# double125/MADTP

Hardware: AMD Instinct MI355X
Metric: images/sec forward, BLIP-base NLVR2 p=0.5 b64; pruned-token index match (higher is better)
Workload: dtype bf16

## Files before the change

madtp_amd/csrc/attention.hip:

```cpp
#include "common.h"
#include "internal.h"
#include <map>
#include <mutex>
#include <stdlib.h>

namespace {

struct AttnArgs {
    const char* q; const char* k; const char* v; char* out; const float* mask;
    float* colsum; float* p0; float* onorm;
    int B, H, Nq, Nk, ldq, ldk, ldv, ldo, nrt;
    float scale;
    const int* kvidx;
    const char* q2; const char* k2; const char* v2; char* out2; const float* mask2; int pair;
    const float* mask_qk; int ld_mqk;
    unsigned* hm_ws; int* hm_tick;
    int kvb;
    float* o_part;
    const int32_t* n_dev;
    int dev_q_only;
    int split_dim; int* range_flag;
};
#define ATTN_DEV_DIMS(a)                                   \
    if ((a).n_dev) {                                       \
// ... 225 lines not shown
    if constexpr (SCORES) {
        if (gridDim.z == 2) {
            const size_t slot = ((size_t)b * gridDim.x + blockIdx.x) * 4 + wave;
            unsigned* mine = a.hm_ws + ((slot * 2 + blockIdx.z) * (2 * HM_MAX_NT)) * 64 + lane;
#pragma unroll
            for (int t = 0; t < NT; ++t)
#pragma unroll
                for (int r = 0; r < 4; ++r)
                    __hip_atomic_store(mine + (4 * t + r) * 64, __float_as_uint(pmax[t][r]), __ATOMIC_RELAXED, __HIP_MEMORY_SCOPE_AGENT);
            asm volatile("s_waitcnt vmcnt(0)" ::: "memory");
            int old = 0;
            if (lane == 0) old = __hip_atomic_fetch_add(a.hm_tick + slot, 1, __ATOMIC_RELAXED, __HIP_MEMORY_SCOPE_AGENT);
            old = __builtin_amdgcn_readfirstlane(old);
            if (old == 0) return;
            if (lane == 0) __hip_atomic_store(a.hm_tick + slot, 0, __ATOMIC_RELAXED, __HIP_MEMORY_SCOPE_AGENT);
            const unsigned* theirs = a.hm_ws + ((slot * 2 + (1 - blockIdx.z)) * (2 * HM_MAX_NT)) * 64 + lane;
#pragma unroll
            for (int t = 0; t < NT; ++t)
#pragma unroll
                for (int r = 0; r < 4; ++r)
                    pmax[t][r] = fmaxf(pmax[t][r], __uint_as_float(__hip_atomic_load(theirs + (4 * t + r) * 64, __ATOMIC_RELAXED,
                                                                                      __HIP_MEMORY_SCOPE_AGENT)));
        }
        if (active) {
            const int i = i0 + l16;
            const bool valid = i >= 1 && i < a.Nq;
            float* dst = a.colsum + ((size_t)b * a.nrt + rt) * a.Nk;
#pragma unroll
            for (int t = 0; t < NT; ++t)
#pragma unroll
                for (int r = 0; r < 4; ++r) {
                    const float v = row16_sum(valid ? pmax[t][r] : 0.f);
                    const int j = 16 * t + 4 * g + r;
                    if (l16 == 0 && j < a.Nk) dst[j] = v;
                }
        }
    }
}

template <int NT, bool SCORES>
__global__ __launch_bounds__(256) void attn_f16s_kernel(AttnArgs a) {
    ATTN_DEV_DIMS(a)
    constexpr int PITCH = NT <= 15 ? 160 : 144;
    constexpr int NKP = NT * 16;
    constexpr int NC = (NT + 1) / 2;
    constexpr int VR = NC * 32;
    extern __shared__ __attribute__((aligned(16))) char smem[];
    char* K0 = smem;
    char* K1 = K0 + NKP * PITCH;
    char* V0 = K1 + NKP * PITCH;
    char* V1 = V0 + VR * PITCH;

    const int tid = threadIdx.x, lane = tid & 63, wave = tid >> 6;
    const int l16 = lane & 15, g = lane >> 4;
    const int b = blockIdx.y;
    const int bkv = a.kvidx ? a.kvidx[b] : b;
    const int rt = blockIdx.x * 4 + wave;
    const int i0 = rt * 16;
    const bool active = i0 < a.Nq;
    const int irow = min(i0 + l16, a.Nq - 1);

    f32x4 pmax[NT];
    if constexpr (SCORES) {
#pragma unroll
        for (int t = 0; t < NT; ++t) pmax[t] = (f32x4){0.f, 0.f, 0.f, 0.f};
    }
    f32x4 mk[NT];
#pragma unroll
    for (int t = 0; t < NT; ++t)
#pragma unroll
        for (int r = 0; r < 4; ++r) {
            const int j = 16 * t + 4 * g + r;
            mk[t][r] = j < a.Nk ? (a.mask ? a.mask[(size_t)b * a.Nk + j] : 0.f) : -INFINITY;
            if (a.mask_qk && j < a.Nk) mk[t][r] += a.mask_qk[(size_t)irow * a.ld_mqk + j];
        }
    if constexpr (VR > NKP) {
        for (int idx = tid; idx < (VR - NKP) * (PITCH / 16); idx += 256) {
            *(uint4*)(V0 + NKP * PITCH + idx * 16) = make_uint4(0, 0, 0, 0);
            *(uint4*)(V1 + NKP * PITCH + idx * 16) = make_uint4(0, 0, 0, 0);
        }
    }

    constexpr int NLD = NT;
    constexpr bool PREFETCH = NLD <= 8;
    uint4 kreg[PREFETCH ? NLD : 1], vreg[PREFETCH ? NLD : 1];
    auto fetch = [&](int h) {
#pragma unroll
        for (int i = 0; i < NLD; ++i) {
            const int idx = tid + 256 * i;
            const int row = idx >> 4, c = idx & 15;
            kreg[i] = make_uint4(0, 0, 0, 0);
            vreg[i] = make_uint4(0, 0, 0, 0);
            if (row < a.Nk) {
                const size_t grow = (size_t)bkv * a.kvb + row;
                kreg[i] = *(const uint4*)(a.k + (grow * a.ldk + h * 64) * 4 + c * 16);
                vreg[i] = *(const uint4*)(a.v + (grow * a.ldv + h * 64) * 4 + c * 16);
            }
        }
    };
    auto put = [&](int idx, uint4 kv, uint4 vv) {
        const int row = idx >> 4, c = idx & 15;
        f16x4 h4, l4;
        split_f16x4(__builtin_bit_cast(f32x4, kv), h4, l4);
        *(f16x4*)(K0 + row * PITCH + c * 8) = h4;
        *(f16x4*)(K1 + row * PITCH + c * 8) = l4;
        split_f16x4(__builtin_bit_cast(f32x4, vv), h4, l4);
        *(f16x4*)(V0 + row * PITCH + c * 8) = h4;
        *(f16x4*)(V1 + row * PITCH + c * 8) = l4;
    };
    if constexpr (PREFETCH) {
        if ((int)blockIdx.z < a.H) fetch(blockIdx.z);
    }
    constexpr float LO = 1.0f / F16S_LO_SCALE;
    for (int h = blockIdx.z; h < a.H; h += gridDim.z) {
        __syncthreads();
        if constexpr (PREFETCH) {
#pragma unroll
            for (int i = 0; i < NLD; ++i) put(tid + 256 * i, kreg[i], vreg[i]);
        } else {
            for (int idx = tid; idx < NKP * 16; idx += 256) {
                const int row = idx >> 4, c = idx & 15;
                uint4 kv = make_uint4(0, 0, 0, 0), vv = make_uint4(0, 0, 0, 0);
                if (row < a.Nk) {
                    const size_t grow = (size_t)bkv * a.kvb + row;
                    kv = *(const uint4*)(a.k + (grow * a.ldk + h * 64) * 4 + c * 16);
                    vv = *(const uint4*)(a.v + (grow * a.ldv + h * 64) * 4 + c * 16);
                }
                put(idx, kv, vv);
            }
        }
        __syncthreads();
        if constexpr (PREFETCH) {
            if (h + (int)gridDim.z < a.H) fetch(h + gridDim.z);
        }
        if (!active) continue;

        f16x8 qh[2], ql[2];
        {
            const char* qp = a.q + (((size_t)b * a.Nq + irow) * a.ldq + h * 64) * 4 + g * 32;
#pragma unroll
            for (int kk = 0; kk < 2; ++kk) {
                u32x4 p0, p1;
                split_f16x8(*(const f32x4*)(qp + kk * 128), *(const f32x4*)(qp + kk * 128 + 16), p0, p1);
                qh[kk] = __builtin_bit_cast(f16x8, p0);
                ql[kk] = __builtin_bit_cast(f16x8, p1);
            }
        }

        f32x4 sc[NT];
#pragma unroll
        for (int t = 0; t < NT; ++t) {
            const int off = (16 * t + l16) * PITCH + g * 16;
            const f16x8 kh0 = *(const f16x8*)(K0 + off), kh1 = *(const f16x8*)(K0 + off + 64);
            const f16x8 kl0 = *(const f16x8*)(K1 + off), kl1 = *(const f16x8*)(K1 + off + 64);
            const f32x4 z = (f32x4){0.f, 0.f, 0.f, 0.f};
            f32x4 hi = __builtin_amdgcn_mfma_f32_16x16x32_f16(kh0, qh[0], z, 0, 0, 0);
            hi = __builtin_amdgcn_mfma_f32_16x16x32_f16(kh1, qh[1], hi, 0, 0, 0);
            f32x4 lo = __builtin_amdgcn_mfma_f32_16x16x32_f16(kh0, ql[0], z, 0, 0, 0);
            lo = __builtin_amdgcn_mfma_f32_16x16x32_f16(kh1, ql[1], lo, 0, 0, 0);
            lo = __builtin_amdgcn_mfma_f32_16x16x32_f16(kl0, qh[0], lo, 0, 0, 0);
            lo = __builtin_amdgcn_mfma_f32_16x16x32_f16(kl1, qh[1], lo, 0, 0, 0);
#pragma unroll
            for (int r = 0; r < 4; ++r) sc[t][r] = fmaf(lo[r], LO, hi[r]);
        }

        float m = -INFINITY;
#pragma unroll
        for (int t = 0; t < NT; ++t)
#pragma unroll
            for (int r = 0; r < 4; ++r) {
                const float v = __fadd_rn(__fmul_rn(sc[t][r], a.scale), mk[t][r]);
                sc[t][r] = v;
                m = fmaxf(m, v);
            }
        m = rows4_max(m);
        float sum = 0.f;
#pragma unroll
        for (int t = 0; t < NT; ++t)
#pragma unroll
            for (int r = 0; r < 4; ++r) {
                const float p = expf(sc[t][r] - m);
                sc[t][r] = p;
                sum += p;
            }
        sum = rows4_sum(sum);
#pragma unroll
        for (int t = 0; t < NT; ++t)
#pragma unroll
            for (int r = 0; r < 4; ++r) {
                const float p = sc[t][r] / sum;
                sc[t][r] = p;
                if constexpr (SCORES) pmax[t][r] = fmaxf(pmax[t][r], p);
            }
        if constexpr (SCORES) {
            if (i0 == 0 && l16 == 0) {
                float* dst = a.p0 + ((size_t)b * a.H + h) * a.Nk;
#pragma unroll
                for (int t = 0; t < NT; ++t)
#pragma unroll
                    for (int r = 0; r < 4; ++r) {
                        const int j = 16 * t + 4 * g + r;
                        if (j < a.Nk) dst[j] = sc[t][r];
                    }
            }
        }

        f32x4 oh[4], ol[4];
#pragma unroll
        for (int dt = 0; dt < 4; ++dt) { oh[dt] = (f32x4){0.f, 0.f, 0.f, 0.f}; ol[dt] = (f32x4){0.f, 0.f, 0.f, 0.f}; }
#pragma unroll
        for (int c = 0; c < NC; ++c) {
            const f32x4 t1 = (2 * c + 1 < NT) ? sc[2 * c + 1 < NT ? 2 * c + 1 : 0] : (f32x4){0.f, 0.f, 0.f, 0.f};
            u32x4 pp0, pp1;
            split_f16x8(sc[2 * c], t1, pp0, pp1);
            const f16x8 ph = __builtin_bit_cast(f16x8, pp0), pl = __builtin_bit_cast(f16x8, pp1);
            const int voff = (32 * c + 4 * g + (l16 >> 2)) * PITCH + 8 * (l16 & 3);
#pragma unroll
            for (int dt = 0; dt < 4; ++dt) {
                const bf16x8 vh = cat_bf16x4(lds_read_tr16(V0 + voff + dt * 32), lds_read_tr16(V0 + voff + 16 * PITCH + dt * 32));
                const bf16x8 vl = cat_bf16x4(lds_read_tr16(V1 + voff + dt * 32), lds_read_tr16(V1 + voff + 16 * PITCH + dt * 32));
                oh[dt] = __builtin_amdgcn_mfma_f32_16x16x32_f16(__builtin_bit_cast(f16x8, vh), ph, oh[dt], 0, 0, 0);
                ol[dt] = __builtin_amdgcn_mfma_f32_16x16x32_f16(__builtin_bit_cast(f16x8, vh), pl, ol[dt], 0, 0, 0);
                ol[dt] = __builtin_amdgcn_mfma_f32_16x16x32_f16(__builtin_bit_cast(f16x8, vl), ph, ol[dt], 0, 0, 0);
            }
        }

        {
            const int i = i0 + l16;
            f32x4 o[4];
            float n2 = 0.f;
#pragma unroll
            for (int dt = 0; dt < 4; ++dt)
#pragma unroll
                for (int r = 0; r < 4; ++r) {
                    o[dt][r] = fmaf(ol[dt][r], LO, oh[dt][r]);
                    n2 += o[dt][r] * o[dt][r];
                }
            if constexpr (SCORES) n2 = rows4_sum(n2);
            if (i < a.Nq) {
                if (a.split_dim) {
                    _Float16* prow = (_Float16*)a.out + ((size_t)b * a.Nq + i) * a.ldo + h * 64 + 4 * g;
                    bool bad = false;
#pragma unroll
                    for (int dt = 0; dt < 4; ++dt) {
                        f16x4 ph_, pl_;
                        split_f16x4(o[dt], ph_, pl_);
                        *(f16x4*)(prow + dt * 16) = ph_;
                        *(f16x4*)(prow + a.split_dim + dt * 16) = pl_;
                        bad |= f16_range_bad(o[dt]);
                    }
                    f16_range_raise(a.range_flag, bad);
                } else {
                    float* orow = (float*)(a.out + (((size_t)b * a.Nq + i) * a.ldo + h * 64) * 4) + 4 * g;
#pragma unroll
                    for (int dt = 0; dt < 4; ++dt) *(f32x4*)(orow + dt * 16) = o[dt];
                }
                if constexpr (SCORES)
                    if (g == 0) a.onorm[((size_t)b * a.H + h) * a.Nq + i] = sqrtf(n2);
            }
        }
    }

    if constexpr (SCORES) {
        if (gridDim.z == 2) {
            const size_t slot = ((size_t)b * gridDim.x + blockIdx.x) * 4 + wave;
            unsigned* mine = a.hm_ws + ((slot * 2 + blockIdx.z) * (2 * HM_MAX_NT)) * 64 + lane;
#pragma unroll
            for (int t = 0; t < NT; ++t)
#pragma unroll
                for (int r = 0; r < 4; ++r)
                    __hip_atomic_store(mine + (4 * t + r) * 64, __float_as_uint(pmax[t][r]), __ATOMIC_RELAXED, __HIP_MEMORY_SCOPE_AGENT);
            asm volatile("s_waitcnt vmcnt(0)" ::: "memory");
            int old = 0;
            if (lane == 0) old = __hip_atomic_fetch_add(a.hm_tick + slot, 1, __ATOMIC_RELAXED, __HIP_MEMORY_SCOPE_AGENT);
            old = __builtin_amdgcn_readfirstlane(old);
            if (old == 0) return;
            if (lane == 0) __hip_atomic_store(a.hm_tick + slot, 0, __ATOMIC_RELAXED, __HIP_MEMORY_SCOPE_AGENT);
            const unsigned* theirs = a.hm_ws + ((slot * 2 + (1 - blockIdx.z)) * (2 * HM_MAX_NT)) * 64 + lane;
#pragma unroll
            for (int t = 0; t < NT; ++t)
#pragma unroll
                for (int r = 0; r < 4; ++r)
                    pmax[t][r] = fmaxf(pmax[t][r], __uint_as_float(__hip_atomic_load(theirs + (4 * t + r) * 64, __ATOMIC_RELAXED,
                                                                                      __HIP_MEMORY_SCOPE_AGENT)));
        }
        if (active) {
            const int i = i0 + l16;
            const bool valid = i >= 1 && i < a.Nq;
            float* dst = a.colsum + ((size_t)b * a.nrt + rt) * a.Nk;
#pragma unroll
            for (int t = 0; t < NT; ++t)
#pragma unroll
                for (int r = 0; r < 4; ++r) {
                    const float v = row16_sum(valid ? pmax[t][r] : 0.f);
                    const int j = 16 * t + 4 * g + r;
                    if (l16 == 0 && j < a.Nk) dst[j] = v;
                }
        }
    }
}

#ifdef MADTP_TS_TIMING
__device__ long long g_attn_dbg[8];
#define AT_MARK(i) do { if (threadIdx.x == 0 && blockIdx.x == 0 && blockIdx.y == 0 && it == 2) { __builtin_amdgcn_s_waitcnt(0); g_attn_dbg[i] = wall_clock64(); } } while (0)
#else
#define AT_MARK(i)
#endif
template <int NT, bool SCORES, int HS, int RB = 1, bool F16 = false>
__global__ __launch_bounds__(256 * HS * RB, (HS == 1 && RB == 1) ? 2 : 1) void attn_bf16_kernel(AttnArgs a) {
    ATTN_DEV_DIMS(a)
    static_assert(HS == 1 || RB == 1, "head-parity split and two row blocks are alternatives");
    constexpr int NKP = NT * 16;
    constexpr int NC = (NT + 1) / 2;
    constexpr int VR = NC * 32;
    constexpr int STAGE = (NKP + VR) * 128;
    extern __shared__ __attribute__((aligned(16))) char smem[];

    const int tid = threadIdx.x, lane = tid & 63;
    const int wave8 = __builtin_amdgcn_readfirstlane(tid >> 6);
    const int wave = wave8 & 3;
    const int hp = HS == 2 ? wave8 >> 2 : 0;
    const int rb = RB == 2 ? wave8 >> 2 : 0;
    constexpr int NSW = 4 * RB;
    const int swave = RB == 2 ? wave8 : wave;
    char* const ring = smem + hp * 2 * STAGE;
    const int l16 = lane & 15, g = lane >> 4;
    int b = blockIdx.y;
    if (a.pair && b >= a.B) {
        b -= a.B;
        a.q = a.q2; a.k = a.k2; a.v = a.v2; a.out = a.out2; a.mask = a.mask2;
    }
    const int bkv = a.kvidx ? a.kvidx[b] : b;
    const int rt = (blockIdx.x * RB + rb) * 4 + wave;
    const int i0 = rt * 16;
    const bool active = i0 < a.Nq;
    const int irow = min(i0 + l16, a.Nq - 1);

    f32x4 pmax[NT];
    if constexpr (SCORES) {
#pragma unroll
        for (int t = 0; t < NT; ++t) pmax[t] = (f32x4){0.f, 0.f, 0.f, 0.f};
    }
    f32x4 mk[NT];
#pragma unroll
    for (int t = 0; t < NT; ++t)
#pragma unroll
        for (int r = 0; r < 4; ++r) {
            const int j = 16 * t + 4 * g + r;
            mk[t][r] = j < a.Nk ? (a.mask ? a.mask[(size_t)b * a.Nk + j] : 0.f) : -INFINITY;
            if (a.mask_qk && j < a.Nk) mk[t][r] += a.mask_qk[(size_t)irow * a.ld_mqk + j];
            mk[t][r] *= 1.44269504088896341f;
        }
    const float c2 = a.scale * 1.44269504088896341f;

    const int sub = lane >> 3, pos = lane & 7;
    constexpr int NDMA = ((NKP + VR) / 8 + NSW - 1) / NSW;
    const char* srcb[NDMA];
#pragma unroll
    for (int i = 0; i < NDMA; ++i) {
        const int grp = swave + NSW * i;
        const bool is_v = grp >= NKP / 8;
        int row = (is_v ? grp - NKP / 8 : grp) * 8 + sub;
        const int chunk = is_v ? (pos ^ (((row >> 1) & 3) << 1)) : (pos ^ (row & 7));
        row = row < a.Nk ? row : a.Nk - 1;
        srcb[i] = (is_v ? a.v + ((size_t)bkv * a.kvb + row) * a.ldv * 2 : a.k + ((size_t)bkv * a.kvb + row) * a.ldk * 2) + chunk * 16;
    }
    auto stage_head = [&](int h, int st) {
        char* base = ring + st * STAGE;
#pragma unroll
        for (int i = 0; i < NDMA; ++i) {
            const int grp = swave + NSW * i;
            if (grp < (NKP + VR) / 8)
                __builtin_amdgcn_global_load_lds(GLOBAL_PTR(srcb[i] + h * 128), LDS_PTR(base + grp * 1024), 16, 0, 0);
        }
    };
    const char* qbase = a.q + ((size_t)b * a.Nq + irow) * a.ldq * 2 + g * 16;
    auto load_q = [&](int h, bf16x8 (&qq)[2]) {
        const char* qp = qbase + h * 128;
        qq[0] = *(const bf16x8*)qp;
        qq[1] = *(const bf16x8*)(qp + 64);
    };
    int st = 0;
    const int hstep = gridDim.z * HS;
    const int hfirst = blockIdx.z * HS + hp;
    const int niter = (a.H - (int)blockIdx.z * HS + hstep - 1) / hstep;
    bf16x8 qn[2];
    if (hfirst < a.H) {
        stage_head(hfirst, 0);
        load_q(hfirst, qn);
    }
    for (int it = 0; it < niter; ++it, st ^= 1) {
        const int h = hfirst + it * hstep;
        bf16x8 q[2] = {qn[0], qn[1]};
        AT_MARK(0);
        __syncthreads();
        AT_MARK(1);
        if (h + hstep < a.H) {
            stage_head(h + hstep, st ^ 1);
            load_q(h + hstep, qn);
        }
        if (!active || h >= a.H) continue;
        AT_MARK(2);
        const char* Ks = ring + st * STAGE;
        const char* Vs = Ks + NKP * 128;

        f32x4 sc[NT];
#pragma unroll
        for (int t = 0; t < NT; ++t) {
            const int row = 16 * t + l16;
            const bf16x8 k0 = *(const bf16x8*)(Ks + row * 128 + (((0 + g) ^ (row & 7)) << 4));
            const bf16x8 k1 = *(const bf16x8*)(Ks + row * 128 + (((4 + g) ^ (row & 7)) << 4));
            f32x4 acc = (f32x4){0.f, 0.f, 0.f, 0.f};
            acc = mfma_lp<F16>(k0, q[0], acc, 0, 0, 0);
            sc[t] = mfma_lp<F16>(k1, q[1], acc, 0, 0, 0);
        }
        AT_MARK(3);
        float m = -INFINITY;
#pragma unroll
        for (int t = 0; t < NT; ++t)
#pragma unroll
            for (int r = 0; r < 4; ++r) {
                const float v = fmaf(sc[t][r], c2, mk[t][r]);
                sc[t][r] = v;
                m = fmaxf(m, v);
            }
        m = rows4_max(m);
        float sum = 0.f;
#pragma unroll
        for (int t = 0; t < NT; ++t)
#pragma unroll
            for (int r = 0; r < 4; ++r) {
                const float p = __builtin_amdgcn_exp2f(sc[t][r] - m);
                sc[t][r] = p;
                sum += p;
            }
        sum = rows4_sum(sum);
        const float inv = __builtin_amdgcn_rcpf(sum);
#pragma unroll
        for (int t = 0; t < NT; ++t) {
            sc[t] *= inv;
            if constexpr (SCORES) {
#pragma unroll
                for (int r = 0; r < 4; ++r) pmax[t][r] = fmaxf(pmax[t][r], sc[t][r]);
            }
        }
        if constexpr (SCORES) {
            if (i0 == 0) {
                if (l16 == 0) {
                    float* dst = a.p0 + ((size_t)b * a.H + h) * a.Nk;
#pragma unroll
                    for (int t = 0; t < NT; ++t)
#pragma unroll
                        for (int r = 0; r < 4; ++r) {
                            const int j = 16 * t + 4 * g + r;
                            if (j < a.Nk) dst[j] = sc[t][r];
                        }
                }
            }
        }
        AT_MARK(4);
        f32x4 o[4];
#pragma unroll
        for (int dt = 0; dt < 4; ++dt) o[dt] = (f32x4){0.f, 0.f, 0.f, 0.f};
#pragma unroll
        for (int c = 0; c < NC; ++c) {
            const f32x4 hi = (2 * c + 1 < NT) ? sc[2 * c + 1 < NT ? 2 * c + 1 : 0] : (f32x4){0.f, 0.f, 0.f, 0.f};
            const bf16x8 pa = pack_lp8<F16>(sc[2 * c], hi);
            const int vrow = 32 * c + 4 * g + (l16 >> 2);
            const int vkey = ((vrow >> 1) & 3) << 1;
            const char* vr = Vs + vrow * 128 + 8 * (l16 & 1);
#pragma unroll
            for (int dt = 0; dt < 4; ++dt) {
                const int p = ((2 * dt + ((l16 & 3) >> 1)) ^ vkey) << 4;
                const bf16x8 vb = cat_bf16x4(lds_read_tr16(vr + p), lds_read_tr16(vr + 16 * 128 + p));
                o[dt] = mfma_lp<F16>(vb, pa, o[dt], 0, 0, 0);
            }
        }
        AT_MARK(5);
        {
            const int i = i0 + l16;
            float n2 = 0.f;
#pragma unroll
            for (int dt = 0; dt < 4; ++dt)
#pragma unroll
                for (int r = 0; r < 4; ++r) n2 += o[dt][r] * o[dt][r];
            if constexpr (SCORES) {
                n2 = rows4_sum(n2);
            }
            if (i < a.Nq) {
                bf16_t* orow = (bf16_t*)(a.out + (((size_t)b * a.Nq + i) * a.ldo + h * 64) * 2) + 4 * g;
#pragma unroll
                for (int dt = 0; dt < 4; ++dt) *(bf16x4*)(orow + dt * 16) = pack_lp4<F16>(o[dt]);
                if constexpr (SCORES)
                    if (g == 0) a.onorm[((size_t)b * a.H + h) * a.Nq + i] = sqrtf(n2);
            }
        }
        AT_MARK(6);
    }

    if constexpr (SCORES && HS == 2) {
        f32x4* xch = (f32x4*)smem;
        __syncthreads();
        if (hp == 1)
#pragma unroll
            for (int t = 0; t < NT; ++t) xch[(wave * NT + t) * 64 + lane] = pmax[t];
        __syncthreads();
        if (hp == 1) return;
#pragma unroll
        for (int t = 0; t < NT; ++t) {
            const f32x4 o = xch[(wave * NT + t) * 64 + lane];
#pragma unroll
            for (int r = 0; r < 4; ++r) pmax[t][r] = fmaxf(pmax[t][r], o[r]);
        }
    }
    if constexpr (SCORES) {
        if (active) {
            const int i = i0 + l16;
            const bool valid = i >= 1 && i < a.Nq;
            float* dst = a.colsum + ((size_t)b * a.nrt + rt) * a.Nk;
#pragma unroll
            for (int t = 0; t < NT; ++t)
#pragma unroll
                for (int r = 0; r < 4; ++r) {
                    const float v = row16_sum(valid ? pmax[t][r] : 0.f);
                    const int j = 16 * t + 4 * g + r;
                    if (l16 == 0 && j < a.Nk) dst[j] = v;
                }
        }
    }
}

constexpr int SMALL_NW = 12;
template <bool F16>
__global__ __launch_bounds__(64 * SMALL_NW, 1) void attn_bf16_small_kernel(AttnArgs a) {
    __shared__ __attribute__((aligned(16))) char vbuf[SMALL_NW][32 * 128];
    __shared__ float pm[SMALL_NW][2][2][64][4];
    const int tid = threadIdx.x, lane = tid & 63;
    const int wave = __builtin_amdgcn_readfirstlane(tid >> 6);
    const int l16 = lane & 15, g = lane >> 4;
    const int b = blockIdx.x;
    const int N = a.Nk;
    char* Vs = vbuf[wave];
    f32x4 pmax[2][2];
#pragma unroll
    for (int rt = 0; rt < 2; ++rt)
#pragma unroll
        for (int t = 0; t < 2; ++t) pmax[rt][t] = (f32x4){0.f, 0.f, 0.f, 0.f};
    const int nrt = (N + 15) / 16;
    f32x4 mk[2];
#pragma unroll
    for (int t = 0; t < 2; ++t)
#pragma unroll
        for (int r = 0; r < 4; ++r) {
            const int j = 16 * t + 4 * g + r;
            mk[t][r] = (j < N ? (a.mask ? a.mask[(size_t)b * N + j] : 0.f) : -INFINITY) * 1.44269504088896341f;
        }
    const float c2 = a.scale * 1.44269504088896341f;

    for (int h = wave; h < a.H; h += SMALL_NW) {
        {
            const int sub = lane >> 3, pos = lane & 7;
#pragma unroll
            for (int grp = 0; grp < 4; ++grp) {
                int row = grp * 8 + sub;
                const int chunk = pos ^ (((row >> 1) & 3) << 1);
                row = row < N ? row : N - 1;
                *(bf16x8*)(Vs + grp * 1024 + lane * 16) =
                    *(const bf16x8*)(a.v + (((size_t)b * N + row) * a.ldv + h * 64) * 2 + chunk * 16);
            }
        }
        bf16x8 kf[2][2];
#pragma unroll
        for (int t = 0; t < 2; ++t) {
            const int j = min(16 * t + l16, N - 1);
            const char* kp = a.k + (((size_t)b * N + j) * a.ldk + h * 64) * 2 + g * 16;
            kf[t][0] = *(const bf16x8*)kp;
            kf[t][1] = *(const bf16x8*)(kp + 64);
        }
#pragma unroll
        for (int rt = 0; rt < 2; ++rt) {
            if (rt >= nrt) break;
            const int i0 = rt * 16;
            const int irow = min(i0 + l16, N - 1);
            const char* qp = a.q + (((size_t)b * N + irow) * a.ldq + h * 64) * 2 + g * 16;
            const bf16x8 q0 = *(const bf16x8*)qp, q1 = *(const bf16x8*)(qp + 64);
            f32x4 sc[2];
            float m = -INFINITY;
#pragma unroll
            for (int t = 0; t < 2; ++t) {
                f32x4 acc = (f32x4){0.f, 0.f, 0.f, 0.f};
                acc = mfma_lp<F16>(kf[t][0], q0, acc, 0, 0, 0);
                acc = mfma_lp<F16>(kf[t][1], q1, acc, 0, 0, 0);
#pragma unroll
                for (int r = 0; r < 4; ++r) {
                    const float v = fmaf(acc[r], c2, mk[t][r]);
                    acc[r] = v;
                    m = fmaxf(m, v);
                }
                sc[t] = acc;
            }
            m = rows4_max(m);
            float sum = 0.f;
#pragma unroll
            for (int t = 0; t < 2; ++t)
#pragma unroll
                for (int r = 0; r < 4; ++r) { sc[t][r] = __builtin_amdgcn_exp2f(sc[t][r] - m); sum += sc[t][r]; }
            sum = rows4_sum(sum);
            const float inv = __builtin_amdgcn_rcpf(sum);
#pragma unroll
            for (int t = 0; t < 2; ++t) {
                sc[t] *= inv;
#pragma unroll
                for (int r = 0; r < 4; ++r) pmax[rt][t][r] = fmaxf(pmax[rt][t][r], sc[t][r]);
            }
            if (i0 == 0) if (l16 == 0) {
                float* dst = a.p0 + ((size_t)b * a.H + h) * N;
#pragma unroll
                for (int t = 0; t < 2; ++t)
#pragma unroll
                    for (int r = 0; r < 4; ++r) {
                        const int j = 16 * t + 4 * g + r;
                        if (j < N) dst[j] = sc[t][r];
                    }
            }
            const bf16x8 pa = pack_lp8<F16>(sc[0], sc[1]);
            const int vrow = 4 * g + (l16 >> 2);
            const int vkey = ((vrow >> 1) & 3) << 1;
            const char* vr = Vs + vrow * 128 + 8 * (l16 & 1);
            f32x4 o[4];
            float n2 = 0.f;
#pragma unroll
            for (int dt = 0; dt < 4; ++dt) {
                const int p = ((2 * dt + ((l16 & 3) >> 1)) ^ vkey) << 4;
                const bf16x8 vb = cat_bf16x4(lds_read_tr16(vr + p), lds_read_tr16(vr + 16 * 128 + p));
                o[dt] = mfma_lp<F16>(vb, pa, (f32x4){0.f, 0.f, 0.f, 0.f}, 0, 0, 0);
#pragma unroll
                for (int r = 0; r < 4; ++r) n2 += o[dt][r] * o[dt][r];
            }
            n2 = rows4_sum(n2);
            const int i = i0 + l16;
            if (i < N) {
                bf16_t* orow = (bf16_t*)(a.out + (((size_t)b * N + i) * a.ldo + h * 64) * 2) + 4 * g;
#pragma unroll
                for (int dt = 0; dt < 4; ++dt) *(bf16x4*)(orow + dt * 16) = pack_lp4<F16>(o[dt]);
                if (g == 0) a.onorm[((size_t)b * a.H + h) * N + i] = sqrtf(n2);
            }
        }
    }
#pragma unroll
    for (int rt = 0; rt < 2; ++rt)
#pragma unroll
        for (int t = 0; t < 2; ++t)
#pragma unroll
            for (int r = 0; r < 4; ++r) pm[wave][rt][t][lane][r] = pmax[rt][t][r];
    __syncthreads();
    if (wave < nrt) {
        const int rt = wave, i = rt * 16 + l16;
        const bool valid = i >= 1 && i < N;
        float* dst = a.colsum + ((size_t)b * a.nrt + rt) * N;
#pragma unroll
        for (int t = 0; t < 2; ++t)
#pragma unroll
            for (int r = 0; r < 4; ++r) {
                float v = pm[0][rt][t][lane][r];
#pragma unroll
                for (int w = 1; w < SMALL_NW; ++w) v = fmaxf(v, pm[w][rt][t][lane][r]);
                v = row16_sum(valid ? v : 0.f);
                const int j = 16 * t + 4 * g + r;
                if (l16 == 0 && j < N) dst[j] = v;
            }
    }
}

template <int NT, bool SCORES, bool F16>
int launch_attn_bf16(const AttnArgs& a, hipStream_t s) {
    constexpr int NC = (NT + 1) / 2;
    constexpr int HS = (SCORES && NT <= 8) ? 2 : 1;
    constexpr int RB = (SCORES && NT > 8) ? 2 : 1;
    const size_t lds = (size_t)2 * HS * (NT * 16 + NC * 32) * 128;
    MADTP_ENSURE_MAX_LDS((attn_bf16_kernel<NT, SCORES, HS, RB, F16>), lds);
    int gz = 1;
    size_t lds_used = lds;
    if (!SCORES) {
        const int wgs = ((a.Nq + 63) / 64) * a.B;
        gz = wgs >= 512 ? 1 : a.H;
        if (gz == a.H) lds_used = lds / 2;
    }
    hipLaunchKernelGGL((attn_bf16_kernel<NT, SCORES, HS, RB, F16>), dim3((a.Nq + 64 * RB - 1) / (64 * RB), (!SCORES && a.pair) ? 2 * a.B : a.B, gz),
                       dim3(256 * HS * RB), lds_used, s, a);
    MADTP_LAUNCH_CHECK();
    return 0;
}

template <bool SCORES, bool F16 = false>
int dispatch_nt_bf16(const AttnArgs& a, hipStream_t s) {
    const int nt = (a.Nk + 15) / 16;
    if (nt <= 4) return launch_attn_bf16<4, SCORES, F16>(a, s);
    if (nt <= 6) return launch_attn_bf16<6, SCORES, F16>(a, s);
    if (nt <= 8) return launch_attn_bf16<8, SCORES, F16>(a, s);
    if (nt <= 10) return launch_attn_bf16<10, SCORES, F16>(a, s);
    if (nt <= 12) return launch_attn_bf16<12, SCORES, F16>(a, s);
    if (nt <= 13) return launch_attn_bf16<13, SCORES, F16>(a, s);
    if (nt <= 16) return launch_attn_bf16<16, SCORES, F16>(a, s);
    return MADTP_E_SHAPE;
}

template <typename T, int NCH, bool SCORES>
__global__ __launch_bounds__(256, 1) void attn_large_kernel(AttnArgs a) {
    constexpr int ESZ = sizeof(T);
    constexpr int RB = 64 * ESZ + 16;
    constexpr int CPR = 64 * ESZ / 16;
    constexpr int CK = 128;
    constexpr int NT = NCH * 8;
    extern __shared__ __attribute__((aligned(16))) char smem[];
    char* Ks = smem;
    char* Vs = smem + CK * RB;

    const int tid = threadIdx.x, lane = tid & 63, wave = tid >> 6;
    const int l16 = lane & 15, g = lane >> 4;
    const int b = blockIdx.y;
    const int bkv = a.kvidx ? a.kvidx[b] : b;
    const int rt = blockIdx.x * 4 + wave;
    const int i0 = rt * 16;
    const bool active = i0 < a.Nq;
    const int irow = min(i0 + l16, a.Nq - 1);

    f32x4 pmax[SCORES ? NT : 1];
    if constexpr (SCORES) {
#pragma unroll
        for (int t = 0; t < NT; ++t) pmax[t] = (f32x4){0.f, 0.f, 0.f, 0.f};
    }

    auto stage = [&](int h, int c, bool with_v) {
        for (int idx = tid; idx < CK * CPR; idx += 256) {
            const int row = idx / CPR, ch = idx % CPR, j = c * CK + row;
            uint4 kv = make_uint4(0, 0, 0, 0), vv = make_uint4(0, 0, 0, 0);
            if (j < a.Nk) {
                const size_t grow = (size_t)bkv * a.kvb + j;
                kv = *(const uint4*)(a.k + (grow * a.ldk + h * 64) * ESZ + ch * 16);
                if (with_v) vv = *(const uint4*)(a.v + (grow * a.ldv + h * 64) * ESZ + ch * 16);
            }
            *(uint4*)(Ks + row * RB + ch * 16) = kv;
            if (with_v) *(uint4*)(Vs + row * RB + ch * 16) = vv;
        }
    };
    auto scores = [&](int c, const f32x4 (&q)[4], f32x4 (&sc)[8]) {
#pragma unroll
        for (int t = 0; t < 8; ++t) sc[t] = (f32x4){0.f, 0.f, 0.f, 0.f};
#pragma unroll
        for (int s = 0; s < 4; ++s) {
            f32x4 kf[8];
#pragma unroll
            for (int t = 0; t < 8; ++t) kf[t] = load4<T>(Ks + (16 * t + l16) * RB + (4 * s + g) * 4 * ESZ);
#pragma unroll
            for (int e = 0; e < 4; ++e)
#pragma unroll
                for (int t = 0; t < 8; ++t) sc[t] = __builtin_amdgcn_mfma_f32_16x16x4f32(kf[t][e], q[s][e], sc[t], 0, 0, 0);
        }
#pragma unroll
        for (int t = 0; t < 8; ++t)
#pragma unroll
            for (int r = 0; r < 4; ++r) {
                const int j = c * CK + 16 * t + 4 * g + r;
                float v = sc[t][r] * a.scale;
                if (a.mask && j < a.Nk) v += a.mask[(size_t)b * a.Nk + j];
                sc[t][r] = j < a.Nk ? v : -INFINITY;
            }
    };

    for (int h = blockIdx.z; h < a.H; h += gridDim.z) {
        f32x4 q[4];
        {
            const char* qp = a.q + (((size_t)b * a.Nq + irow) * a.ldq + h * 64) * ESZ;
#pragma unroll
            for (int s = 0; s < 4; ++s) q[s] = load4<T>(qp + (4 * s + g) * 4 * ESZ);
        }
        float m = -INFINITY, l = 0.f;
        for (int c = 0; c < NCH; ++c) {
            if (c * CK >= a.Nk) break;
            __syncthreads();
            stage(h, c, false);
            __syncthreads();
            if (!active) continue;
            f32x4 sc[8];
            scores(c, q, sc);
            float cm = -INFINITY;
#pragma unroll
            for (int t = 0; t < 8; ++t)
#pragma unroll
                for (int r = 0; r < 4; ++r) cm = fmaxf(cm, sc[t][r]);
            cm = rows4_max(cm);
            const float mn = fmaxf(m, cm);
            float cs = 0.f;
#pragma unroll
            for (int t = 0; t < 8; ++t)
#pragma unroll
                for (int r = 0; r < 4; ++r) cs += expf(sc[t][r] - mn);
            cs = rows4_sum(cs);
            l = l * expf(m - mn) + cs;
            m = mn;
        }
        f32x4 o[4];
#pragma unroll
        for (int dt = 0; dt < 4; ++dt) o[dt] = (f32x4){0.f, 0.f, 0.f, 0.f};
#pragma unroll
        for (int c = 0; c < NCH; ++c) {
            if (c * CK < a.Nk) {
                __syncthreads();
                stage(h, c, true);
                __syncthreads();
                if (active) {
                    f32x4 sc[8];
                    scores(c, q, sc);
#pragma unroll
                    for (int t = 0; t < 8; ++t) {
#pragma unroll
                        for (int r = 0; r < 4; ++r) {
                            const float p = expf(sc[t][r] - m) / l;
                            sc[t][r] = p;
                            if constexpr (SCORES) pmax[c * 8 + t][r] = fmaxf(pmax[c * 8 + t][r], p);
                        }
                    }
                    if constexpr (SCORES) {
                        if (i0 + l16 == 0) {
                            float* dst = a.p0 + ((size_t)b * a.H + h) * a.Nk;
#pragma unroll
                            for (int t = 0; t < 8; ++t)
#pragma unroll
                                for (int r = 0; r < 4; ++r) {
                                    const int j = c * CK + 16 * t + 4 * g + r;
                                    if (j < a.Nk) dst[j] = sc[t][r];
                                }
                        }
                    }
#pragma unroll
                    for (int t = 0; t < 8; ++t)
#pragma unroll
                        for (int r = 0; r < 4; ++r) {
                            const char* vrow = Vs + (16 * t + 4 * g + r) * RB + l16 * ESZ;
#pragma unroll
                            for (int dt = 0; dt < 4; ++dt)
                                o[dt] = __builtin_amdgcn_mfma_f32_16x16x4f32(sc[t][r], load1<T>(vrow + dt * 16 * ESZ), o[dt], 0, 0, 0);
                        }
                }
            }
        }
        if (active) {
#pragma unroll
            for (int r = 0; r < 4; ++r) {
                const int i = i0 + 4 * g + r;
                float n2 = 0.f;
#pragma unroll
                for (int dt = 0; dt < 4; ++dt) n2 += o[dt][r] * o[dt][r];
                if constexpr (SCORES) n2 = row16_sum(n2);
                if (i < a.Nq) {
                    T* orow = (T*)(a.out + (((size_t)b * a.Nq + i) * a.ldo + h * 64) * ESZ);
#pragma unroll
                    for (int dt = 0; dt < 4; ++dt) orow[dt * 16 + l16] = from_f32<T>(o[dt][r]);
                    if constexpr (SCORES)
                        if (l16 == 0) a.onorm[((size_t)b * a.H + h) * a.Nq + i] = sqrtf(n2);
                }
            }
        }
    }
    if constexpr (SCORES) {
        if (active) {
            const int i = i0 + l16;
            const bool valid = i >= 1 && i < a.Nq;
            float* dst = a.colsum + ((size_t)b * a.nrt + rt) * a.Nk;
#pragma unroll
            for (int t = 0; t < NT; ++t)
#pragma unroll
                for (int r = 0; r < 4; ++r) {
                    const float v = row16_sum(valid ? pmax[t][r] : 0.f);
                    const int j = 16 * t + 4 * g + r;
                    if (l16 == 0 && j < a.Nk) dst[j] = v;
                }
        }
    }
}

template <int NCH, bool SCORES>
__global__ __launch_bounds__(256, 1) void attn_large_f16s_kernel(AttnArgs a) {
    constexpr int PITCH = 160;
    constexpr int CK = 128;
    constexpr int NT = NCH * 8;
    extern __shared__ __attribute__((aligned(16))) char smem[];
    char* K0 = smem;
    char* K1 = K0 + CK * PITCH;
    char* V0 = K1 + CK * PITCH;
    char* V1 = V0 + CK * PITCH;

    const int tid = threadIdx.x, lane = tid & 63, wave = tid >> 6;
    const int l16 = lane & 15, g = lane >> 4;
    const int b = blockIdx.y;
    const int bkv = a.kvidx ? a.kvidx[b] : b;
    const int rt = blockIdx.x * 4 + wave;
    const int i0 = rt * 16;
    const bool active = i0 < a.Nq;
    const int irow = min(i0 + l16, a.Nq - 1);
    constexpr float LO = 1.0f / F16S_LO_SCALE;

    f32x4 pmax[SCORES ? NT : 1];
    if constexpr (SCORES) {
#pragma unroll
        for (int t = 0; t < NT; ++t) pmax[t] = (f32x4){0.f, 0.f, 0.f, 0.f};
    }

    auto stage = [&](int h, int c, bool with_v) {
#pragma unroll
        for (int half = 0; half < 2; ++half) {
            uint4 kr[4], vr[4];
#pragma unroll
            for (int i = 0; i < 4; ++i) {
                const int idx = tid + 256 * (4 * half + i), row = idx >> 4, ch = idx & 15, j = c * CK + row;
                kr[i] = make_uint4(0, 0, 0, 0);
                vr[i] = make_uint4(0, 0, 0, 0);
                if (j < a.Nk) {
                    const size_t grow = (size_t)bkv * a.kvb + j;
                    kr[i] = *(const uint4*)(a.k + (grow * a.ldk + h * 64) * 4 + ch * 16);
                    if (with_v) vr[i] = *(const uint4*)(a.v + (grow * a.ldv + h * 64) * 4 + ch * 16);
                }
            }
#pragma unroll
            for (int i = 0; i < 4; ++i) {
                const int idx = tid + 256 * (4 * half + i), row = idx >> 4, ch = idx & 15;
                f16x4 h4, l4;
                split_f16x4(__builtin_bit_cast(f32x4, kr[i]), h4, l4);
                *(f16x4*)(K0 + row * PITCH + ch * 8) = h4;
                *(f16x4*)(K1 + row * PITCH + ch * 8) = l4;
                if (with_v) {
                    split_f16x4(__builtin_bit_cast(f32x4, vr[i]), h4, l4);
                    *(f16x4*)(V0 + row * PITCH + ch * 8) = h4;
                    *(f16x4*)(V1 + row * PITCH + ch * 8) = l4;
                }
            }
        }
    };
    auto scores = [&](int c, const f16x8 (&qh)[2], const f16x8 (&ql)[2], f32x4 (&sc)[8]) {
#pragma unroll
        for (int t = 0; t < 8; ++t) {
            const int off = (16 * t + l16) * PITCH + g * 16;
            const f16x8 kh0 = *(const f16x8*)(K0 + off), kh1 = *(const f16x8*)(K0 + off + 64);
            const f16x8 kl0 = *(const f16x8*)(K1 + off), kl1 = *(const f16x8*)(K1 + off + 64);
            const f32x4 z = (f32x4){0.f, 0.f, 0.f, 0.f};
            f32x4 hi = __builtin_amdgcn_mfma_f32_16x16x32_f16(kh0, qh[0], z, 0, 0, 0);
            hi = __builtin_amdgcn_mfma_f32_16x16x32_f16(kh1, qh[1], hi, 0, 0, 0);
            f32x4 lo = __builtin_amdgcn_mfma_f32_16x16x32_f16(kh0, ql[0], z, 0, 0, 0);
            lo = __builtin_amdgcn_mfma_f32_16x16x32_f16(kh1, ql[1], lo, 0, 0, 0);
            lo = __builtin_amdgcn_mfma_f32_16x16x32_f16(kl0, qh[0], lo, 0, 0, 0);
            lo = __builtin_amdgcn_mfma_f32_16x16x32_f16(kl1, qh[1], lo, 0, 0, 0);
#pragma unroll
            for (int r = 0; r < 4; ++r) {
                const int j = c * CK + 16 * t + 4 * g + r;
                float v = fmaf(lo[r], LO, hi[r]) * a.scale;
                if (a.mask && j < a.Nk) v += a.mask[(size_t)b * a.Nk + j];
                sc[t][r] = j < a.Nk ? v : -INFINITY;
            }
        }
    };

    for (int h = blockIdx.z; h < a.H; h += gridDim.z) {
        f16x8 qh[2], ql[2];
        {
            const char* qp = a.q + (((size_t)b * a.Nq + irow) * a.ldq + h * 64) * 4 + g * 32;
#pragma unroll
            for (int kk = 0; kk < 2; ++kk) {
                u32x4 p0, p1;
                split_f16x8(*(const f32x4*)(qp + kk * 128), *(const f32x4*)(qp + kk * 128 + 16), p0, p1);
                qh[kk] = __builtin_bit_cast(f16x8, p0);
                ql[kk] = __builtin_bit_cast(f16x8, p1);
            }
        }
        float m = -INFINITY, l = 0.f;
        for (int c = 0; c < NCH; ++c) {
            if (c * CK >= a.Nk) break;
            __syncthreads();
            stage(h, c, false);
            __syncthreads();
            if (!active) continue;
            f32x4 sc[8];
            scores(c, qh, ql, sc);
// ... 925 lines not shown
```

Measured before the change: 26340.

## Pipeline V LDS reads and defer output stores in scoring attention head loop

Adds an NL variant of the bf16 attention kernel for the scoring path, enabled by default through an env flag. It double-buffers the transposed V reads from LDS across chunks using inline ds_read_b64_tr_b16 with explicit waitcnt. It also defers each head's output and norm store until after the next iteration's barrier, so global writes overlap the next head's work. The __syncthreads is replaced by an explicit waitcnt plus s_barrier. The inline asm and manual wait counts add correctness and scheduling risk, and the held results raise register pressure.

```diff
diff --git a/madtp_amd/csrc/attention.hip b/madtp_amd/csrc/attention.hip
--- a/madtp_amd/csrc/attention.hip
+++ b/madtp_amd/csrc/attention.hip
@@ -551,11 +551,11 @@
 
 #ifdef MADTP_TS_TIMING
 __device__ long long g_attn_dbg[8];
-#define AT_MARK(i) do { if (threadIdx.x == 0 && blockIdx.x == 0 && blockIdx.y == 0 && it == 2) { __builtin_amdgcn_s_waitcnt(0); g_attn_dbg[i] = wall_clock64(); } } while (0)
+#define AT_MARK(i) do { if (threadIdx.x == 0 && blockIdx.x == 0 && blockIdx.y == 0 && it == 2) { if (!NL) __builtin_amdgcn_s_waitcnt(0); g_attn_dbg[i] = wall_clock64(); } } while (0)
 #else
 #define AT_MARK(i)
 #endif
-template <int NT, bool SCORES, int HS, int RB = 1, bool F16 = false>
+template <int NT, bool SCORES, int HS, int RB = 1, bool F16 = false, bool NL = false>
 __global__ __launch_bounds__(256 * HS * RB, (HS == 1 && RB == 1) ? 2 : 1) void attn_bf16_kernel(AttnArgs a) {
     ATTN_DEV_DIMS(a)
     static_assert(HS == 1 || RB == 1, "head-parity split and two row blocks are alternatives");
@@ -638,12 +638,38 @@
         stage_head(hfirst, 0);
         load_q(hfirst, qn);
     }
+    auto store_o = [&](int hh, const bf16x4 (&pk)[4], float nrm) {
+        const int i = i0 + l16;
+        if (i < a.Nq) {
+            bf16_t* orow = (bf16_t*)(a.out + (((size_t)b * a.Nq + i) * a.ldo + hh * 64) * 2) + 4 * g;
+#pragma unroll
+            for (int dt = 0; dt < 4; ++dt) *(bf16x4*)(orow + dt * 16) = pk[dt];
+            if constexpr (SCORES)
+                if (g == 0) a.onorm[((size_t)b * a.H + hh) * a.Nq + i] = nrm;
+        }
+    };
+    bf16x4 po[4];
+    float pn = 0.f;
+    bool pend = false;
     for (int it = 0; it < niter; ++it, st ^= 1) {
         const int h = hfirst + it * hstep;
         bf16x8 q[2] = {qn[0], qn[1]};
         AT_MARK(0);
-        __syncthreads();
+        if constexpr (NL) {
+            __builtin_amdgcn_sched_barrier(0);
+            asm volatile("s_waitcnt vmcnt(0) lgkmcnt(0)" : "+v"(q[0]), "+v"(q[1]) :: "memory");
+            __builtin_amdgcn_s_barrier();
+            __builtin_amdgcn_sched_barrier(0);
+        } else {
+            __syncthreads();
+        }
         AT_MARK(1);
+        if constexpr (NL) {
+            if (pend) {
+                store_o(h - hstep, po, pn);
+                pend = false;
+            }
+        }
         if (h + hstep < a.H) {
             stage_head(h + hstep, st ^ 1);
             load_q(h + hstep, qn);
@@ -711,6 +737,32 @@
         f32x4 o[4];
 #pragma unroll
         for (int dt = 0; dt < 4; ++dt) o[dt] = (f32x4){0.f, 0.f, 0.f, 0.f};
+        if constexpr (NL) {
+            bf16x4 vt[2][8];
+            auto v_reads = [&](int c, bf16x4 (&d)[8]) {
+                const int vrow = 32 * c + 4 * g + (l16 >> 2);
+                const int vkey = ((vrow >> 1) & 3) << 1;
+                const char* vr = Vs + vrow * 128 + 8 * (l16 & 1);
+#pragma unroll
+                for (int dt = 0; dt < 4; ++dt) {
+                    const unsigned ad = (unsigned)(uintptr_t)(__attribute__((address_space(3))) const char*)(vr + (((2 * dt + ((l16 & 3) >> 1)) ^ vkey) << 4));
+                    asm volatile("ds_read_b64_tr_b16 %0, %1" : "=v"(d[2 * dt]) : "v"(ad) : "memory");
+                    asm volatile("ds_read_b64_tr_b16 %0, %1 offset:2048" : "=v"(d[2 * dt + 1]) : "v"(ad) : "memory");
+                }
+            };
+            v_reads(0, vt[0]);
+#pragma unroll
+            for (int c = 0; c < NC; ++c) {
+                const f32x4 hi = (2 * c + 1 < NT) ? sc[2 * c + 1 < NT ? 2 * c + 1 : 0] : (f32x4){0.f, 0.f, 0.f, 0.f};
+                const bf16x8 pa = pack_lp8<F16>(sc[2 * c], hi);
+                asm volatile("s_waitcnt lgkmcnt(0)" : "+v"(vt[c & 1][0]), "+v"(vt[c & 1][1]), "+v"(vt[c & 1][2]), "+v"(vt[c & 1][3]),
+                             "+v"(vt[c & 1][4]), "+v"(vt[c & 1][5]), "+v"(vt[c & 1][6]), "+v"(vt[c & 1][7]) :: "memory");
+#pragma unroll
+                for (int dt = 0; dt < 4; ++dt)
+                    o[dt] = mfma_lp<F16>(cat_bf16x4(vt[c & 1][2 * dt], vt[c & 1][2 * dt + 1]), pa, o[dt], 0, 0, 0);
+                if (c + 1 < NC) v_reads(c + 1, vt[(c + 1) & 1]);
+            }
+        } else
 #pragma unroll
         for (int c = 0; c < NC; ++c) {
             const f32x4 hi = (2 * c + 1 < NT) ? sc[2 * c + 1 < NT ? 2 * c + 1 : 0] : (f32x4){0.f, 0.f, 0.f, 0.f};
@@ -736,7 +788,12 @@
             if constexpr (SCORES) {
                 n2 = rows4_sum(n2);
             }
-            if (i < a.Nq) {
+            if constexpr (NL) {
+#pragma unroll
+                for (int dt = 0; dt < 4; ++dt) po[dt] = pack_lp4<F16>(o[dt]);
+                pn = sqrtf(n2);
+                pend = true;
+            } else if (i < a.Nq) {
                 bf16_t* orow = (bf16_t*)(a.out + (((size_t)b * a.Nq + i) * a.ldo + h * 64) * 2) + 4 * g;
 #pragma unroll
                 for (int dt = 0; dt < 4; ++dt) *(bf16x4*)(orow + dt * 16) = pack_lp4<F16>(o[dt]);
@@ -745,6 +802,9 @@
             }
         }
         AT_MARK(6);
+    }
+    if constexpr (NL) {
+        if (pend) store_o(hfirst + (niter - 1) * hstep, po, pn);
     }
 
     if constexpr (SCORES && HS == 2) {
@@ -927,6 +987,16 @@
     constexpr int HS = (SCORES && NT <= 8) ? 2 : 1;
     constexpr int RB = (SCORES && NT > 8) ? 2 : 1;
     const size_t lds = (size_t)2 * HS * (NT * 16 + NC * 32) * 128;
+    if constexpr (SCORES) {
+        static int headloop_env = -1;
+        if (headloop_env < 0) { const char* e = getenv("MADTP_ATTN_HEADLOOP"); headloop_env = e ? atoi(e) != 0 : 1; }
+        if (headloop_env) {
+            MADTP_ENSURE_MAX_LDS((attn_bf16_kernel<NT, true, HS, RB, F16, true>), lds);
+            hipLaunchKernelGGL((attn_bf16_kernel<NT, true, HS, RB, F16, true>), dim3((a.Nq + 64 * RB - 1) / (64 * RB), a.B, 1), dim3(256 * HS * RB), lds, s, a);
+            MADTP_LAUNCH_CHECK();
+            return 0;
+        }
+    }
     MADTP_ENSURE_MAX_LDS((attn_bf16_kernel<NT, SCORES, HS, RB, F16>), lds);
     int gz = 1;
     size_t lds_used = lds;
```

New measurement: 26120. No clear change (-0.8%).
